# tanishqkumar/ssd

Measured on AMD Instinct MI355X. Metric: output tokens/sec + p50 TTFT, Llama-3-70B SSD k=7 f=3; mean accepted len, higher is better.
Workload: dtype bf16

## Files before the change

### ssd_amd/csrc/gemm_pf.hip

```cpp
#include "common.h"
#include <algorithm>
#include <cstdlib>

enum { PF_EPI_ROWS = 0, PF_EPI_SILU_FRAG = 1, PF_EPI_PARTIALS = 2 };

constexpr int PF_WAVES_DEFAULT = 4;
constexpr int PF_U = 4;

template <int MT, int NT, int UU, int DIRECT, int PF_WAVES, int BPS = 1, int BPRE = 0>
__global__ void __launch_bounds__(64 * PF_WAVES, PF_WAVES <= 4 ? 2 : 1)
gemm_pf_kernel(const u32x4_t* __restrict__ Wf, const u32x4_t* __restrict__ Xf, float* __restrict__ ws,
               int M, int N, int K, int kt_per_split, int mt_valid, const bf16_t* __restrict__ bias,
               void* __restrict__ Yv, int ldy) {
  __shared__ u32x4_t xs[2 * BPS][MT][64];
  constexpr int KTS = 16 + DIRECT;
  KTRACE(KTS, 0);
  constexpr int U = UU;
  static_assert(UU % (2 * BPS) == 0, "an even number of phases per unrolled pass");
  constexpr int FPW = (MT + PF_WAVES - 1) / PF_WAVES;
  const int lane = threadIdx.x & 63;
  const int wave = __builtin_amdgcn_readfirstlane(threadIdx.x >> 6);
  const int KT = K >> 5;
  const int g0 = (blockIdx.x * PF_WAVES + wave) * NT;
  const int kz0 = blockIdx.y * kt_per_split;
  const int nk = kt_per_split;

  f32x4_t acc[NT][MT];
#pragma unroll
  for (int nt = 0; nt < NT; ++nt)
#pragma unroll
    for (int mt = 0; mt < MT; ++mt) acc[nt][mt] = f32x4_t{0.f, 0.f, 0.f, 0.f};

  const u32x4_t* wp = Wf + (((size_t)g0 * KT + kz0) << 6) + lane;
  const size_t wstride = (size_t)KT << 6;
  const u32x4_t* xp[FPW];
  int xmt[FPW];
#pragma unroll
  for (int f = 0; f < FPW; ++f) {
    xmt[f] = wave + PF_WAVES * f;
    const int src = min(xmt[f], mt_valid - 1);
    xp[f] = Xf + (((size_t)src * KT + kz0) << 6) + lane;
  }

  u32x4_t a[U][NT], xr[2][BPS][FPW];
  auto load_w = [&](u32x4_t (&d)[NT], int kt) {
#pragma unroll
    for (int nt = 0; nt < NT; ++nt) d[nt] = __builtin_nontemporal_load(wp + nt * wstride + ((size_t)kt << 6));
  };
  auto load_x = [&](u32x4_t (&d)[FPW], int kt) {
#pragma unroll
    for (int f = 0; f < FPW; ++f) d[f] = xp[f][(size_t)kt << 6];
  };
  auto stage_x = [&](const u32x4_t (&d)[FPW], int slot) {
#pragma unroll
    for (int f = 0; f < FPW; ++f)
      if (xmt[f] < MT) xs[slot][xmt[f]][lane] = d[f];
  };
  auto compute = [&](const u32x4_t (&w)[NT], int slot) {
#pragma unroll
    for (int mt = 0; mt < MT; ++mt) {
      const u32x4_t b = xs[slot][mt][lane];
#pragma unroll
      for (int nt = 0; nt < NT; ++nt) acc[nt][mt] = mfma16(w[nt], b, acc[nt][mt]);
    }
  };

  const int klast = nk - 1;
#pragma unroll
  for (int b = 0; b < BPS; ++b) load_x(xr[0][b], b);
#pragma unroll
  for (int u = 0; u < U; ++u) load_w(a[u], u);
#pragma unroll
  for (int b = 0; b < BPS; ++b) load_x(xr[1][b], BPS + b);
#pragma unroll
  for (int b = 0; b < BPS; ++b) stage_x(xr[0][b], b);
#pragma unroll
  for (int b = 0; b < BPS; ++b) load_x(xr[0][b], min(2 * BPS + b, klast));
  KTRACE(KTS, 1);
  __syncthreads();
  KTRACE(KTS, 2);
  for (int kt = 0; kt < nk; kt += U) {
#pragma unroll
    for (int u = 0; u < U; u += BPS) {
      const int k = kt + u;
      const int par = (u / BPS) & 1;
#pragma unroll
      for (int b = 0; b < BPS; ++b) stage_x(xr[par ^ 1][b], (par ^ 1) * BPS + b);
#pragma unroll
      for (int b = 0; b < BPS; ++b) load_x(xr[par ^ 1][b], min(k + 3 * BPS + b, klast));
      if constexpr (BPRE == 2 && BPS == 2) {
        u32x4_t b0[MT], b1[MT];
#pragma unroll
        for (int mt = 0; mt < MT; ++mt) b0[mt] = xs[par * BPS][mt][lane];
#pragma unroll
        for (int mt = 0; mt < MT; ++mt) b1[mt] = xs[par * BPS + 1][mt][lane];
        __builtin_amdgcn_sched_barrier(0);
#pragma unroll
        for (int mt = 0; mt < MT; ++mt)
#pragma unroll
          for (int nt = 0; nt < NT; ++nt) acc[nt][mt] = mfma16(a[u][nt], b0[mt], acc[nt][mt]);
        load_w(a[u], min(k + U, klast));
#pragma unroll
        for (int mt = 0; mt < MT; ++mt)
#pragma unroll
          for (int nt = 0; nt < NT; ++nt) acc[nt][mt] = mfma16(a[u + 1][nt], b1[mt], acc[nt][mt]);
        load_w(a[u + 1], min(k + 1 + U, klast));
      } else {
#pragma unroll
        for (int b = 0; b < BPS; ++b) {
          compute(a[u + b], par * BPS + b);
          load_w(a[u + b], min(k + b + U, klast));
        }
      }
      __syncthreads();
    }
  }

  KTRACE(KTS, 3);
  const int mcol = lane & 15, nrow = (lane >> 4) * 4;
  if constexpr (DIRECT == 1) {
#pragma unroll
    for (int nt = 0; nt < NT; ++nt) {
      const int n = (g0 + nt) * 16 + nrow;
#pragma unroll
      for (int mt = 0; mt < MT; ++mt) {
        const int m = mt * 16 + mcol;
        f32x4_t s = acc[nt][mt];
        if (bias) {
#pragma unroll
          for (int r = 0; r < 4; ++r) s[r] += bf2f(bias[n + r]);
        }
        if (m < M) {
          const u32x2_t v = {pack_bf2(s[0], s[1]), pack_bf2(s[2], s[3])};
          *reinterpret_cast<u32x2_t*>(reinterpret_cast<bf16_t*>(Yv) + (size_t)m * ldy + n) = v;
        }
      }
    }
    KTRACE(KTS, 4);
    return;
  }
  if constexpr (DIRECT == 2) {
    const int KT2 = (N >> 1) >> 5;
    u32x2_t* out2 = reinterpret_cast<u32x2_t*>(Yv);
#pragma unroll
    for (int pr = 0; pr < NT / 2; ++pr) {
      const int f = ((g0 >> 1) + pr) * 16 + nrow;
      const int ng = (g0 + 2 * pr) * 16 + nrow, nu = ng + 16;
#pragma unroll
      for (int mt = 0; mt < MT; ++mt) {
        const int m = mt * 16 + mcol;
        float o[4];
#pragma unroll
        for (int r = 0; r < 4; ++r) {
          float gb = acc[2 * pr][mt][r], ub = acc[2 * pr + 1][mt][r];
          if (bias) { gb += bf2f(bias[ng + r]); ub += bf2f(bias[nu + r]); }
          gb = round_bf(gb); ub = round_bf(ub);
          o[r] = (gb / (1.0f + __expf(-gb))) * ub;
        }
        if (m < M) {
          const u32x2_t v = {pack_bf2(o[0], o[1]), pack_bf2(o[2], o[3])};
          out2[frag_chunk(m, f >> 3, KT2) * 2 + ((f >> 2) & 1)] = v;
        }
      }
    }
    KTRACE(KTS, 4);
    return;
  }
  float* out = ws + (size_t)blockIdx.y * M * N;
#pragma unroll
  for (int nt = 0; nt < NT; ++nt) {
    const int n = (g0 + nt) * 16 + nrow;
#pragma unroll
    for (int mt = 0; mt < MT; ++mt) {
      const int m = mt * 16 + mcol;
      if (m < M) *reinterpret_cast<f32x4_t*>(out + (size_t)m * N + n) = acc[nt][mt];
    }
  }
  KTRACE(KTS, 4);
}

template <int EPI>
__global__ void __launch_bounds__(256)
gemm_pf_epilogue_kernel(const float* __restrict__ ws, const bf16_t* __restrict__ bias, void* __restrict__ Yv,
                        int M, int N, int splits, int ldy) {
  const size_t MN = (size_t)M * N;
  if (EPI == PF_EPI_ROWS) {
    const size_t i4 = ((size_t)blockIdx.x * blockDim.x + threadIdx.x) * 4;
    if (i4 >= MN) return;
    const int m = (int)(i4 / N), n = (int)(i4 % N);
    f32x4_t s = *reinterpret_cast<const f32x4_t*>(ws + i4);
    for (int z = 1; z < splits; ++z) s += *reinterpret_cast<const f32x4_t*>(ws + z * MN + i4);
    if (bias) {
#pragma unroll
      for (int r = 0; r < 4; ++r) s[r] += bf2f(bias[n + r]);
    }
    const u32x2_t v = {pack_bf2(s[0], s[1]), pack_bf2(s[2], s[3])};
    *reinterpret_cast<u32x2_t*>(reinterpret_cast<bf16_t*>(Yv) + (size_t)m * ldy + n) = v;
  } else {
    const int half = N >> 1;
    const size_t i4 = ((size_t)blockIdx.x * blockDim.x + threadIdx.x) * 4;
    if (i4 >= (size_t)M * half) return;
    const int m = (int)(i4 / half), f = (int)(i4 % half);
    const int ng = ((f >> 4) * 2) * 16 + (f & 15), nu = ng + 16;
    f32x4_t g = *reinterpret_cast<const f32x4_t*>(ws + (size_t)m * N + ng);
    f32x4_t u = *reinterpret_cast<const f32x4_t*>(ws + (size_t)m * N + nu);
    for (int z = 1; z < splits; ++z) {
      g += *reinterpret_cast<const f32x4_t*>(ws + z * MN + (size_t)m * N + ng);
      u += *reinterpret_cast<const f32x4_t*>(ws + z * MN + (size_t)m * N + nu);
    }
    float o[4];
#pragma unroll
    for (int r = 0; r < 4; ++r) {
      float gb = g[r], ub = u[r];
      if (bias) { gb += bf2f(bias[ng + r]); ub += bf2f(bias[nu + r]); }
      gb = round_bf(gb); ub = round_bf(ub);
      o[r] = (gb / (1.0f + __expf(-gb))) * ub;
    }
    const u32x2_t v = {pack_bf2(o[0], o[1]), pack_bf2(o[2], o[3])};
    reinterpret_cast<u32x2_t*>(Yv)[frag_chunk(m, f >> 3, half >> 5) * 2 + ((f >> 2) & 1)] = v;
  }
}

template <int MT, int NT, int DIRECT>
static int pf_launch_d(const void* x, const void* w, float* ws, int M, int N, int K, int splits, const void* bias, void* y,
                       int ldy, int waves, int uu, int bps, int bpre, hipStream_t st) {
  const int KT = K >> 5;
  dim3 grid(N / (16 * NT * waves), splits);
  const int nk = KT / splits;
  if (uu <= 0) uu = (NT <= 2 && nk % 8 == 0) ? 8 : PF_U;
  if (nk % uu != 0 || bps < 1) return SSD_ERR_ARG;
  bool launched = false;
#define PF_GO_B(UU, WV, B, PRE)                                                                                          \
  if (!launched && uu == UU && waves == WV && bps == B && bpre == PRE) {                                                 \
    launched = true;                                                                                                     \
    hipLaunchKernelGGL((gemm_pf_kernel<MT, NT, UU, DIRECT, WV, B, PRE>), grid, dim3(64 * WV), 0, st, (const u32x4_t*)w, \
                       (const u32x4_t*)x, ws, M, N, K, nk, (M + 15) / 16, (const bf16_t*)bias, y, ldy);                  \
  }
#define PF_GO(UU, WV, B) PF_GO_B(UU, WV, B, 0)
  PF_GO(4, 4, 1)
  if constexpr (NT == 1 && MT == 8 && DIRECT != 2) {
    PF_GO(8, 4, 1) PF_GO(8, 4, 2) PF_GO(8, 8, 1) PF_GO(8, 8, 2)
  }
  if constexpr (NT == 2) {
    PF_GO(8, 4, 1) PF_GO(4, 8, 1) PF_GO(8, 8, 1)
    if constexpr (MT == 8) {
      PF_GO(8, 4, 2) PF_GO(8, 8, 2)
      PF_GO_B(8, 4, 2, 2) PF_GO_B(8, 8, 2, 2) PF_GO_B(8, 5, 2, 2)
      PF_GO(8, 3, 1) PF_GO(8, 3, 2) PF_GO(8, 5, 1) PF_GO(8, 5, 2) PF_GO(8, 6, 2) PF_GO(8, 7, 1) PF_GO(8, 7, 2)
    }
  }
#undef PF_GO
#undef PF_GO_B
  if (!launched) return SSD_ERR_ARG;
  return hipGetLastError() == hipSuccess ? SSD_OK : SSD_ERR_LAUNCH;
}

template <int MT, int NT>
static int pf_launch(const void* x, const void* w, float* ws, int M, int N, int K, int splits, int direct, const void* bias,
                     void* y, int ldy, int waves, int uu, int bps, int bpre, hipStream_t st) {
  if (direct == 1) return pf_launch_d<MT, NT, 1>(x, w, ws, M, N, K, splits, bias, y, ldy, waves, uu, bps, bpre, st);
  if (direct == 2) return pf_launch_d<MT, NT, 2>(x, w, ws, M, N, K, splits, bias, y, ldy, waves, uu, bps, bpre, st);
  return pf_launch_d<MT, NT, 0>(x, w, ws, M, N, K, splits, bias, y, ldy, waves, uu, bps, bpre, st);
}

static void pf_pick(int N, int K, int* nt_out, int* splits_out, int* waves_out = nullptr) {
  const int KT = K >> 5;
  int nt = 2, waves = 4, s = 1;
  if (N % (16 * 2 * 4) != 0) { *nt_out = 4; *splits_out = 1; if (waves_out) *waves_out = 4; return; }
  const int blocks4 = N / (16 * 2 * 4);
  if (blocks4 < 160) {
    while (s < 8 && (blocks4 * s < 160 || KT / s > 96)) s *= 2;
    while (s > 1 && KT % (s * PF_U) != 0) s /= 2;
  }
  if (N % (16 * 2 * 8) == 0 && (N / (16 * 2 * 8)) * s >= 160) waves = 8;
  *nt_out = nt; *splits_out = s;
  if (waves_out) *waves_out = waves;
}

static void pf_refine(int M, int N, int K, int splits, int* waves, int* bps) {
  *bps = 1;
  if (M <= 64) return;
  const int nk = (K >> 5) / splits;
  if (nk % 8 != 0) return;
  *bps = 2;
  if (N % (16 * 2 * 5) == 0 && ((N / (16 * 2 * 5)) * splits) % 256 == 0) *waves = 5;
}

typedef __attribute__((address_space(1))) void* lm_gptr_t;
typedef __attribute__((address_space(3))) void* lm_lptr_t;
constexpr int LM_MAX_M = 16384;
constexpr int LM_CUS = 256;

template <int BM, int BN, int WM, int WN, int DIRECT>
__global__ void __launch_bounds__(64 * WM * WN, 1)
gemm_lm_kernel(const u32x4_t* __restrict__ Wf, const u32x4_t* __restrict__ Xf, float* __restrict__ ws, int M, int N, int K,
               int nkb, int tiles_m, int tiles_n, const bf16_t* __restrict__ bias, void* __restrict__ Yv, int ldy) {
  constexpr int NW = WM * WN;
  constexpr int TW = BN / 16, TX = BM / 16, TT = TW + TX;
  constexpr int G = 2 * TT / NW;
  constexpr int MTW = TX / WM, NTW = TW / WN;
  static_assert((2 * TT) % NW == 0 && TX % WM == 0 && TW % WN == 0 && NTW % 2 == 0, "tile geometry");
  __shared__ u32x4_t lds[2][2][TT][64];
  const int lane = threadIdx.x & 63;
  const int wave = __builtin_amdgcn_readfirstlane(threadIdx.x >> 6);
  const int wm = wave / WN, wn = wave % WN;
  const int KT = K >> 5;

  const int nwg = gridDim.x, orig = blockIdx.x;
  const int q = nwg >> 3, r = nwg & 7, xcd = orig & 7;
  const int wgid = (xcd < r ? xcd * (q + 1) : r * (q + 1) + (xcd - r) * q) + (orig >> 3);
  const int tiles = tiles_m * tiles_n;
  const int z = wgid / tiles, t = wgid - z * tiles;
  const int mg0 = (t % tiles_m) * TX, ng0 = (t / tiles_m) * TW;
  const int mg_valid = (M + 15) >> 4, ng_valid = N >> 4;
  const int kt0 = z * nkb * 2;

  const u32x4_t* src[G];
#pragma unroll
  for (int i = 0; i < G; ++i) {
    const int j = wave * G + i, tt = j % TT, ks = j / TT;
    const int grp = tt < TW ? min(ng0 + tt, ng_valid - 1) : min(mg0 + tt - TW, mg_valid - 1);
    src[i] = (tt < TW ? Wf : Xf) + (((size_t)grp * KT + kt0 + ks) << 6) + lane;
  }
  auto issue = [&](int kb, int buf) {
#pragma unroll
    for (int i = 0; i < G; ++i) {
      const int j = wave * G + i;
      __builtin_amdgcn_global_load_lds((lm_gptr_t)(src[i] + ((size_t)kb << 7)), (lm_lptr_t)&lds[buf][j / TT][j % TT][0], 16, 0, 0);
    }
  };

  f32x4_t acc[NTW][MTW];
#pragma unroll
  for (int nt = 0; nt < NTW; ++nt)
#pragma unroll
    for (int mt = 0; mt < MTW; ++mt) acc[nt][mt] = f32x4_t{0.f, 0.f, 0.f, 0.f};

  issue(0, 0);
  for (int kb = 0; kb < nkb; ++kb) {
    const int cur = kb & 1;
    asm volatile("s_waitcnt vmcnt(0) lgkmcnt(0)" ::: "memory");
    __builtin_amdgcn_s_barrier();
    asm volatile("" ::: "memory");
    if (kb + 1 < nkb) issue(kb + 1, cur ^ 1);
#pragma unroll
    for (int ks = 0; ks < 2; ++ks) {
      u32x4_t a[NTW], b[MTW];
#pragma unroll
      for (int nt = 0; nt < NTW; ++nt) a[nt] = lds[cur][ks][wn * NTW + nt][lane];
#pragma unroll
      for (int mt = 0; mt < MTW; ++mt) b[mt] = lds[cur][ks][TW + wm * MTW + mt][lane];
#pragma unroll
      for (int mt = 0; mt < MTW; ++mt)
#pragma unroll
        for (int nt = 0; nt < NTW; ++nt) acc[nt][mt] = mfma16(a[nt], b[mt], acc[nt][mt]);
    }
  }

  const int mcol = lane & 15, nrow = (lane >> 4) * 4;
  const int gm0 = mg0 + wm * MTW, gn0 = ng0 + wn * NTW;
  if constexpr (DIRECT == 1) {
#pragma unroll
    for (int nt = 0; nt < NTW; ++nt) {
      if (gn0 + nt >= ng_valid) continue;
      const int n = (gn0 + nt) * 16 + nrow;
      float bv[4] = {0.f, 0.f, 0.f, 0.f};
      if (bias) {
#pragma unroll
        for (int r4 = 0; r4 < 4; ++r4) bv[r4] = bf2f(bias[n + r4]);
      }
#pragma unroll
      for (int mt = 0; mt < MTW; ++mt) {
        const int m = (gm0 + mt) * 16 + mcol;
        f32x4_t s = acc[nt][mt];
        if (bias) {
#pragma unroll
          for (int r4 = 0; r4 < 4; ++r4) s[r4] += bv[r4];
        }
        if (m < M) {
          const u32x2_t v = {pack_bf2(s[0], s[1]), pack_bf2(s[2], s[3])};
          *reinterpret_cast<u32x2_t*>(reinterpret_cast<bf16_t*>(Yv) + (size_t)m * ldy + n) = v;
        }
      }
    }
  } else if constexpr (DIRECT == 2) {
    const int KT2 = (N >> 1) >> 5;
    u32x2_t* out2 = reinterpret_cast<u32x2_t*>(Yv);
#pragma unroll
    for (int pr = 0; pr < NTW / 2; ++pr) {
      const int gg = gn0 + 2 * pr;
      if (gg >= ng_valid) continue;
      const int f = (gg >> 1) * 16 + nrow;
      const int ng = gg * 16 + nrow, nu = ng + 16;
#pragma unroll
      for (int mt = 0; mt < MTW; ++mt) {
        const int m = (gm0 + mt) * 16 + mcol;
        float o[4];
#pragma unroll
        for (int r4 = 0; r4 < 4; ++r4) {
          float gb = acc[2 * pr][mt][r4], ub = acc[2 * pr + 1][mt][r4];
          if (bias) { gb += bf2f(bias[ng + r4]); ub += bf2f(bias[nu + r4]); }
          gb = round_bf(gb); ub = round_bf(ub);
          o[r4] = (gb / (1.0f + __expf(-gb))) * ub;
        }
        if (m < M) {
          const u32x2_t v = {pack_bf2(o[0], o[1]), pack_bf2(o[2], o[3])};
          out2[frag_chunk(m, f >> 3, KT2) * 2 + ((f >> 2) & 1)] = v;
        }
      }
    }
  } else {
    float* out = ws + (size_t)z * M * N;
#pragma unroll
    for (int nt = 0; nt < NTW; ++nt) {
      if (gn0 + nt >= ng_valid) continue;
      const int n = (gn0 + nt) * 16 + nrow;
#pragma unroll
      for (int mt = 0; mt < MTW; ++mt) {
        const int m = (gm0 + mt) * 16 + mcol;
        if (m < M) *reinterpret_cast<f32x4_t*>(out + (size_t)m * N + n) = acc[nt][mt];
      }
    }
  }
}

constexpr int LM_FORMS = 4;
static const int lm_bm[LM_FORMS] = {256, 128, 256, 128}, lm_bn[LM_FORMS] = {256, 256, 128, 128}, lm_occ[LM_FORMS] = {1, 1, 1, 2};

static int64_t lm_tiles(int form, int M, int N) {
  return (int64_t)((M + lm_bm[form] - 1) / lm_bm[form]) * ((N + lm_bn[form] - 1) / lm_bn[form]);
}

static void lm_pick(int M, int N, int K, int* form_out, int* splits_out) {
  static const double rel[LM_FORMS] = {1.0, 0.8, 0.8, 0.8};
  int best = 0;
  double best_t = 0;
  for (int f = 0; f < LM_FORMS; ++f) {
    const int64_t per_round = (int64_t)LM_CUS * lm_occ[f];
    const double t = (double)((lm_tiles(f, M, N) + per_round - 1) / per_round) * lm_bm[f] * lm_bn[f] * lm_occ[f] / (65536.0 * rel[f]);
    if (f == 0 || t < best_t - 1e-9) { best = f; best_t = t; }
  }
  const int64_t cnt = lm_tiles(best, M, N), slots = (int64_t)LM_CUS * lm_occ[best];
  const int nkb = K / 64;
  int s = 1;
  if (cnt * 2 <= slots)
    while (s < 8 && cnt * s * 2 <= slots && nkb % (s * 2) == 0 && nkb / (s * 2) >= 8) s *= 2;
  *form_out = best + 1;
  *splits_out = s;
}

static int64_t lm_workspace(int M, int N, int K) {
  int form, s;
  lm_pick(M, N, K, &form, &s);
  return s > 1 ? (int64_t)s * M * N * 4 : 0;
}

template <int BM, int BN, int WM, int WN>
static int lm_go(const void* x, const void* w, float* ws, int M, int N, int K, int splits, int direct, const void* bias, void* y,
                 int ldy, hipStream_t st) {
  const int tiles_m = (M + BM - 1) / BM, tiles_n = (N + BN - 1) / BN;
  const int nkb = (K / 64) / splits;
  const dim3 grid((unsigned)(tiles_m * tiles_n * splits)), block(64 * WM * WN);
#define LM_ARGS (const u32x4_t*)w, (const u32x4_t*)x, ws, M, N, K, nkb, tiles_m, tiles_n, (const bf16_t*)bias, y, ldy
  if (direct == 1) hipLaunchKernelGGL((gemm_lm_kernel<BM, BN, WM, WN, 1>), grid, block, 0, st, LM_ARGS);
  else if (direct == 2) hipLaunchKernelGGL((gemm_lm_kernel<BM, BN, WM, WN, 2>), grid, block, 0, st, LM_ARGS);
  else hipLaunchKernelGGL((gemm_lm_kernel<BM, BN, WM, WN, 0>), grid, block, 0, st, LM_ARGS);
#undef LM_ARGS
  return hipGetLastError() == hipSuccess ? SSD_OK : SSD_ERR_LAUNCH;
}

static int lm_gemm(const void* x_frag, const void* w_frag, const void* bias, void* y, int M, int N, int K, int ldy, int epilogue,
                   void* workspace, int64_t workspace_bytes, int form, int splits, hipStream_t st) {
  if (M > LM_MAX_M || N <= 0 || K <= 0 || N % 128 != 0 || K % 128 != 0) return SSD_ERR_SHAPE;
  if (epilogue != PF_EPI_ROWS && epilogue != PF_EPI_SILU_FRAG) return SSD_ERR_ARG;
  if (form < 0 || form > LM_FORMS) return SSD_ERR_ARG;
  int dform, dsplits;
  lm_pick(M, N, K, &dform, &dsplits);
  if (form == 0) form = dform;
  if (splits <= 0) splits = dform == form ? dsplits : 1;
  if (splits > 16 || (K / 64) % splits != 0) return SSD_ERR_ARG;
  if (!x_frag || !w_frag || !y) return SSD_ERR_ARG;
  const int direct = splits == 1 ? (epilogue == PF_EPI_ROWS ? 1 : 2) : 0;
  if (!direct && (!workspace || workspace_bytes < (int64_t)splits * M * N * 4)) return SSD_ERR_ARG;
  float* ws = (float*)workspace;
  int rc;
#define LM_A x_frag, w_frag, ws, M, N, K, splits, direct, bias, y, ldy, st
  switch (form) {
    case 1: rc = lm_go<256, 256, 2, 4>(LM_A); break;
    case 2: rc = lm_go<128, 256, 2, 4>(LM_A); break;
    case 3: rc = lm_go<256, 128, 4, 2>(LM_A); break;
    default: rc = lm_go<128, 128, 2, 2>(LM_A); break;
  }
#undef LM_A
  if (rc != SSD_OK || direct) return rc;
  if (epilogue == PF_EPI_ROWS) {
    const size_t items = (size_t)M * N / 4;
    hipLaunchKernelGGL((gemm_pf_epilogue_kernel<PF_EPI_ROWS>), dim3((unsigned)((items + 255) / 256)), dim3(256), 0, st, ws,
                       (const bf16_t*)bias, y, M, N, splits, ldy);
  } else {
    const size_t items = (size_t)M * (N / 2) / 4;
    hipLaunchKernelGGL((gemm_pf_epilogue_kernel<PF_EPI_SILU_FRAG>), dim3((unsigned)((items + 255) / 256)), dim3(256), 0, st, ws,
                       (const bf16_t*)bias, y, M, N, splits, ldy);
  }
  return hipGetLastError() == hipSuccess ? SSD_OK : SSD_ERR_LAUNCH;
}

extern "C" int ssd_gemm_pf_workspace_bytes(int M, int N, int K, int64_t* bytes) {
  if (!bytes || M <= 0 || N <= 0 || K <= 0 || N % (16 * 2 * PF_WAVES_DEFAULT) != 0) return SSD_ERR_ARG;
  if (M > 128) {
    if (M > LM_MAX_M || K % 128 != 0) return SSD_ERR_ARG;
    int64_t need = 0;
    for (int m = 256;; m += 128) {
      const int mm = m < M ? m : M;
      need = std::max(need, lm_workspace(mm, N, K));
      if (mm == M) break;
    }
    *bytes = need;
    return SSD_OK;
  }
  int nt, splits;
  pf_pick(N, K, &nt, &splits);
  *bytes = (int64_t)splits * M * N * 4;
  return SSD_OK;
}

extern "C" int ssd_gemm_pf_cfg(const void* x_frag, const void* w_frag, const void* bias, void* y, int M, int N, int K,
                               int ldy, int epilogue, void* workspace, int64_t workspace_bytes, int nt, int splits,
                               void* stream) {
  if (M > 128) return lm_gemm(x_frag, w_frag, bias, y, M, N, K, ldy, epilogue, workspace, workspace_bytes, nt & 0xff, splits,
                              (hipStream_t)stream);
  if (M <= 16 || M > 128 || N <= 0 || K <= 0 || (K % (32 * PF_U))) return SSD_ERR_SHAPE;
  if (epilogue != PF_EPI_ROWS && epilogue != PF_EPI_SILU_FRAG && epilogue != PF_EPI_PARTIALS) return SSD_ERR_ARG;
  if (epilogue == PF_EPI_PARTIALS && bias) return SSD_ERR_ARG;
  int waves = (nt >> 8) & 0xff;
  const int uu = (nt >> 16) & 0xff;
  int bps = (nt >> 24) & 0xf;
  const int bpre = (nt >> 28) & 3;
  nt &= 0xff;
  if (waves == 0) waves = PF_WAVES_DEFAULT;
  if (bps == 0) bps = 1;
  if (nt != 1 && nt != 2 && nt != 4) return SSD_ERR_ARG;
  if (nt == 1 && (epilogue == PF_EPI_SILU_FRAG || M <= 64)) return SSD_ERR_ARG;
  if (waves != 4 && !(waves >= 3 && waves <= 8 && nt <= 2)) return SSD_ERR_ARG;
  if (N % (16 * nt * waves) != 0) return SSD_ERR_SHAPE;
  const int KT = K >> 5;
  if (splits <= 0) { int nt_d; pf_pick(N, K, &nt_d, &splits); if (nt_d != nt) splits = 1; }
  if (splits > 16) return SSD_ERR_ARG;
  if (KT % (splits * PF_U) != 0) return SSD_ERR_ARG;
  const int direct = (splits == 1 && epilogue != PF_EPI_PARTIALS) ? (epilogue == PF_EPI_ROWS ? 1 : 2) : 0;
  if (!direct && (!workspace || workspace_bytes < (int64_t)splits * M * N * 4)) return SSD_ERR_ARG;
  hipStream_t st = (hipStream_t)stream;
  float* ws = (float*)workspace;
  const int mt = (M + 15) / 16;
  int rc;
#define PF_ARGS x_frag, w_frag, ws, M, N, K, splits, direct, bias, y, ldy, waves, uu, bps, bpre, st
  if (mt <= 4) rc = nt == 4 ? pf_launch<4, 4>(PF_ARGS) : pf_launch<4, 2>(PF_ARGS);
  else rc = nt == 4 ? pf_launch<8, 4>(PF_ARGS) : nt == 2 ? pf_launch<8, 2>(PF_ARGS) : pf_launch<8, 1>(PF_ARGS);
#undef PF_ARGS
  if (rc != SSD_OK || direct || epilogue == PF_EPI_PARTIALS) return rc;
  if (epilogue == PF_EPI_ROWS) {
    const size_t items = (size_t)M * N / 4;
    hipLaunchKernelGGL((gemm_pf_epilogue_kernel<PF_EPI_ROWS>), dim3((unsigned)((items + 255) / 256)), dim3(256), 0, st, ws,
                       (const bf16_t*)bias, y, M, N, splits, ldy);
  } else {
    const size_t items = (size_t)M * (N / 2) / 4;
    hipLaunchKernelGGL((gemm_pf_epilogue_kernel<PF_EPI_SILU_FRAG>), dim3((unsigned)((items + 255) / 256)), dim3(256), 0, st,
                       ws, (const bf16_t*)bias, y, M, N, splits, ldy);
  }
  return hipGetLastError() == hipSuccess ? SSD_OK : SSD_ERR_LAUNCH;
}

extern "C" int ssd_gemm_pf(const void* x_frag, const void* w_frag, const void* bias, void* y, int M, int N, int K,
                           int ldy, int epilogue, void* workspace, int64_t workspace_bytes, int splits, void* stream) {
  if (N <= 0 || K <= 0 || N % (16 * 2 * PF_WAVES_DEFAULT) != 0) return SSD_ERR_SHAPE;
  if (M > 128) return lm_gemm(x_frag, w_frag, bias, y, M, N, K, ldy, epilogue, workspace, workspace_bytes, 0, splits, (hipStream_t)stream);
  int nt, s, waves, bps;
  pf_pick(N, K, &nt, &s, &waves);
  if (splits > 0) { s = splits; waves = 4; }
  if (s > 16 || (K >> 5) % s != 0) return SSD_ERR_ARG;
  pf_refine(M, N, K, s, &waves, &bps);
  const int bpre = (bps == 2 && nt == 2 && M > 64 && (waves == 4 || waves == 5 || waves == 8) && ((K >> 5) / s) % 8 == 0) ? 2 : 0;
  return ssd_gemm_pf_cfg(x_frag, w_frag, bias, y, M, N, K, ldy, epilogue, workspace, workspace_bytes,
                         nt | (waves << 8) | (bps << 24) | (bpre << 28), s, stream);
}

KT_DEFINE_SETTER(gemm_pf)
```

Measured before the change: 113.0.

## Add streaming multi-stage LDS ring GEMM kernel for under-occupied skinny GEMMs

Adds a new gemm_ps kernel that streams weight and activation tiles into a deep shared-memory ring buffer using direct global-to-LDS loads, with explicit vmcnt waits to keep several stages in flight. The default path now routes to it when the old config launches too few workgroups, choosing a tile width so the workgroup count is a multiple of the CU count. The intent is to raise memory-level parallelism and CU fill for bandwidth-bound small-M GEMMs. The epilogue store is also factored into a shared helper, and a probe script is added. The hand-tuned waitcnt accounting and the new shape selection could lower performance or break correctness on some shapes.

```diff
diff --git a/profiles/pf_stream_probe.py b/profiles/pf_stream_probe.py
--- /dev/null
+++ b/profiles/pf_stream_probe.py
@@ -0,0 +1,124 @@
+import argparse
+import ctypes as C
+import json
+import os
+import sys
+
+import torch
+
+ROOT = os.path.dirname(os.path.dirname(os.path.abspath(__file__)))
+sys.path.insert(0, ROOT)
+import ssd_amd.hip.lib as L
+
+if os.environ.get("SSD_PROBE_LIB"):
+    L.lib_path = lambda: os.environ["SSD_PROBE_LIB"]
+from ssd_amd.hip import ops as H
+
+BF = torch.bfloat16
+STREAM = 1 << 30
+SHAPES = [
+    ("70b.qkv", 10240, 8192, H.EPI_ROWS), ("70b.o", 8192, 8192, H.PF_EPI_PARTIALS),
+    ("70b.gate_up", 57344, 8192, H.EPI_SILU_FRAG), ("70b.down", 8192, 28672, H.PF_EPI_PARTIALS),
+    ("8b.gate_up", 28672, 4096, H.EPI_SILU_FRAG), ("8b.down", 4096, 14336, H.PF_EPI_PARTIALS),
+    ("qwen32b.qkv", 10240, 5120, H.EPI_ROWS), ("qwen32b.gate_up", 51200, 5120, H.EPI_SILU_FRAG),
+    ("qwen32b.down", 5120, 25600, H.PF_EPI_PARTIALS),
+]
+
+
+def old_default(M, N, K):
+    KT = K >> 5
+    waves, s = 4, 1
+    blocks4 = N // 128
+    if blocks4 < 160:
+        while s < 8 and (blocks4 * s < 160 or KT // s > 96):
+            s *= 2
+        while s > 1 and KT % (s * 4) != 0:
+            s //= 2
+    if N % 256 == 0 and (N // 256) * s >= 160:
+        waves = 8
+    bps = 1
+    if M > 64 and (KT // s) % 8 == 0:
+        bps = 2
+        if N % 160 == 0 and ((N // 160) * s) % 256 == 0:
+            waves = 5
+    bpre = 2 if (bps == 2 and M > 64 and waves in (4, 5, 8)) else 0
+    return 2 | (waves << 8) | (bps << 24) | (bpre << 28), s
+
+
+def call(lib, xf, w, y, ws, M, N, K, epi, nt, splits):
+    rc = lib.ssd_gemm_pf_cfg(xf.data_ptr(), w.data_ptr(), None, y.data_ptr(), M, N, K, N, epi, ws.data_ptr(),
+                             ws.numel() * 4, nt, splits, C.c_void_p(torch.cuda.current_stream().cuda_stream))
+    return rc
+
+
+def out_bytes(y, ws, M, N, epi, splits):
+    if epi == H.PF_EPI_PARTIALS:
+        return ws[: splits * M * N].view(torch.int32).clone()
+    return y.view(torch.int16).clone()
+
+
+@torch.inference_mode()
+def main():
+    ap = argparse.ArgumentParser()
+    ap.add_argument("--reps", type=int, default=20)
+    ap.add_argument("--m", type=int, nargs="+", default=[128])
+    ap.add_argument("--lm", action="store_true")
+    ap.add_argument("--shapes", nargs="+", default=None)
+    a = ap.parse_args()
+    lib = L.load_library()
+    lib.ssd_gemm_pf_cfg.restype = C.c_int
+    lib.ssd_gemm_pf_cfg.argtypes = [C.c_void_p, C.c_void_p, C.c_void_p, C.c_void_p, C.c_int, C.c_int, C.c_int, C.c_int, C.c_int,
+                                    C.c_void_p, C.c_int64, C.c_int, C.c_int, C.c_void_p]
+    for name, N, K, epi in SHAPES:
+        if a.shapes and name not in a.shapes:
+            continue
+        nbuf = max(3, -(-(2 << 30) // (2 * N * K)))
+        ws_ = [(torch.randn(N * K // 64, device="cuda") * 0.05).to(BF).repeat(64) for _ in range(nbuf)]
+        for M in a.m:
+            xf = (torch.randn(H.frag_numel(M, K), device="cuda") * 0.5).to(BF)
+            y = torch.zeros(M * N, device="cuda", dtype=BF)
+            wsb = torch.zeros(16 * M * N + 64, dtype=torch.float32, device="cuda")
+            nt0, s0 = old_default(M, N, K)
+            forms = [("old", nt0, s0)]
+            for tw in (16, 14, 12, 10, 8, 6):
+                if N % (16 * tw) == 0:
+                    forms.append((f"stream.tw{tw}", STREAM | (tw << 8), s0))
+                    if M > 64:
+                        forms.append((f"stream.tw{tw}.kpb1", STREAM | (tw << 8) | (1 << 24), s0))
+            forms.append(("default", None, 0))
+            if a.lm and M == 128:
+                forms += [("lm.128x256", (1 << 31) | 2, s0), ("lm.128x128", (1 << 31) | 4, s0)]
+            ref = None
+            for fname, nt, s in forms:
+                def go(i):
+                    if nt is None:
+                        H.gemm_pf(xf, ws_[i % nbuf], y, M, N, K, N, wsb, epilogue=epi)
+                        return 0
+                    return call(lib, xf, ws_[i % nbuf], y, wsb, M, N, K, epi, C.c_int32(nt & 0xffffffff).value, s)
+                y.zero_(); wsb.zero_()
+                rc = go(0)
+                if rc != 0:
+                    print(json.dumps({"matrix": name, "M": M, "form": fname, "rc": rc}), flush=True)
+                    continue
+                torch.cuda.synchronize()
+                got = out_bytes(y, wsb, M, N, epi, s0)
+                if ref is None:
+                    ref = got
+                same = bool(torch.equal(got, ref))
+                for i in range(3):
+                    go(i)
+                ev = [(torch.cuda.Event(enable_timing=True), torch.cuda.Event(enable_timing=True)) for _ in range(a.reps)]
+                for i, (e0, e1) in enumerate(ev):
+                    e0.record(); go(i + 1); e1.record()
+                torch.cuda.synchronize()
+                t = sorted(e0.elapsed_time(e1) * 1e3 for e0, e1 in ev)
+                us = t[len(t) // 2]
+                print(json.dumps({"matrix": name, "N": N, "K": K, "M": M, "form": fname, "nt": nt, "splits": s0, "us_p50": round(us, 1),
+                                  "us_min": round(t[0], 1), "tb_s": round(2 * N * K / us / 1e6, 2), "bit_identical_to_old": same}),
+                      flush=True)
+        del ws_
+        torch.cuda.empty_cache()
+
+
+if __name__ == "__main__":
+    main()
diff --git a/ssd_amd/csrc/gemm_pf.hip b/ssd_amd/csrc/gemm_pf.hip
--- a/ssd_amd/csrc/gemm_pf.hip
+++ b/ssd_amd/csrc/gemm_pf.hip
@@ -6,6 +6,66 @@
 
 constexpr int PF_WAVES_DEFAULT = 4;
 constexpr int PF_U = 4;
+
+template <int MT, int NT, int DIRECT>
+__device__ __forceinline__ void pf_store(const f32x4_t (&acc)[NT][MT], int g0, int lane, int M, int N, float* __restrict__ ws,
+                                         int z, const bf16_t* __restrict__ bias, void* __restrict__ Yv, int ldy) {
+  const int mcol = lane & 15, nrow = (lane >> 4) * 4;
+  if constexpr (DIRECT == 1) {
+#pragma unroll
+    for (int nt = 0; nt < NT; ++nt) {
+      const int n = (g0 + nt) * 16 + nrow;
+#pragma unroll
+      for (int mt = 0; mt < MT; ++mt) {
+        const int m = mt * 16 + mcol;
+        f32x4_t s = acc[nt][mt];
+        if (bias) {
+#pragma unroll
+          for (int r = 0; r < 4; ++r) s[r] += bf2f(bias[n + r]);
+        }
+        if (m < M) {
+          const u32x2_t v = {pack_bf2(s[0], s[1]), pack_bf2(s[2], s[3])};
+          *reinterpret_cast<u32x2_t*>(reinterpret_cast<bf16_t*>(Yv) + (size_t)m * ldy + n) = v;
+        }
+      }
+    }
+  } else if constexpr (DIRECT == 2) {
+    const int KT2 = (N >> 1) >> 5;
+    u32x2_t* out2 = reinterpret_cast<u32x2_t*>(Yv);
+#pragma unroll
+    for (int pr = 0; pr < NT / 2; ++pr) {
+      const int f = ((g0 >> 1) + pr) * 16 + nrow;
+      const int ng = (g0 + 2 * pr) * 16 + nrow, nu = ng + 16;
+#pragma unroll
+      for (int mt = 0; mt < MT; ++mt) {
+        const int m = mt * 16 + mcol;
+        float o[4];
+#pragma unroll
+        for (int r = 0; r < 4; ++r) {
+          float gb = acc[2 * pr][mt][r], ub = acc[2 * pr + 1][mt][r];
+          if (bias) { gb += bf2f(bias[ng + r]); ub += bf2f(bias[nu + r]); }
+          gb = round_bf(gb); ub = round_bf(ub);
+          o[r] = (gb / (1.0f + __expf(-gb))) * ub;
+        }
+        if (m < M) {
+          const u32x2_t v = {pack_bf2(o[0], o[1]), pack_bf2(o[2], o[3])};
+          out2[frag_chunk(m, f >> 3, KT2) * 2 + ((f >> 2) & 1)] = v;
+        }
+      }
+    }
+  } else {
+    float* out = ws + (size_t)z * M * N;
+#pragma unroll
+    for (int nt = 0; nt < NT; ++nt) {
+      const int n = (g0 + nt) * 16 + nrow;
+#pragma unroll
+      for (int mt = 0; mt < MT; ++mt) {
+        const int m = mt * 16 + mcol;
+        if (m < M) *reinterpret_cast<f32x4_t*>(out + (size_t)m * N + n) = acc[nt][mt];
+      }
+    }
+  }
+}
 
 template <int MT, int NT, int UU, int DIRECT, int PF_WAVES, int BPS = 1, int BPRE = 0>
 __global__ void __launch_bounds__(64 * PF_WAVES, PF_WAVES <= 4 ? 2 : 1)
@@ -117,65 +177,107 @@
   }
 
   KTRACE(KTS, 3);
-  const int mcol = lane & 15, nrow = (lane >> 4) * 4;
-  if constexpr (DIRECT == 1) {
-#pragma unroll
-    for (int nt = 0; nt < NT; ++nt) {
-      const int n = (g0 + nt) * 16 + nrow;
+  pf_store<MT, NT, DIRECT>(acc, g0, lane, M, N, ws, blockIdx.y, bias, Yv, ldy);
+  KTRACE(KTS, 4);
+}
+
+typedef __attribute__((address_space(1))) void* lm_gptr_t;
+typedef __attribute__((address_space(3))) void* lm_lptr_t;
+
+template <int MT, int TW, int KPB>
+struct PsGeom {
+  static constexpr int NW = TW / 2;
+  static constexpr int TT = TW + MT;
+  static constexpr int ST = 160 / TT < 8 ? 160 / TT : 8;
+  static constexpr int XPW = (MT + NW - 1) / NW;
+  static constexpr int L = 2 + XPW;
+  static constexpr int VM_STEADY = (ST - 2 * KPB) * L;
+  static_assert(TW % 2 == 0 && ST >= 2 * KPB + 1 && VM_STEADY <= 63, "stream geometry");
+};
+
+template <int MT, int TW, int DIRECT, int KPB>
+__global__ void __launch_bounds__(32 * TW, 1)
+gemm_ps_kernel(const u32x4_t* __restrict__ Wf, const u32x4_t* __restrict__ Xf, float* __restrict__ ws,
+               int M, int N, int K, int nk, int mt_valid, const bf16_t* __restrict__ bias, void* __restrict__ Yv, int ldy) {
+  using G = PsGeom<MT, TW, KPB>;
+  constexpr int NW = G::NW, TT = G::TT, ST = G::ST, XPW = G::XPW;
+  __shared__ u32x4_t ring[ST][TT][64];
+  constexpr int KTS = 19 + DIRECT;
+  KTRACE(KTS, 0);
+  const int lane = threadIdx.x & 63;
+  const int wave = __builtin_amdgcn_readfirstlane(threadIdx.x >> 6);
+  const int KT = K >> 5;
+  const int g0 = (blockIdx.x * NW + wave) * 2;
+  const int kz0 = blockIdx.y * nk;
+
+  const u32x4_t* wsrc = Wf + (((size_t)g0 * KT + kz0) << 6) + lane;
+  const size_t wstride = (size_t)KT << 6;
+  const u32x4_t* xsrc[XPW];
+  int xslot[XPW];
+#pragma unroll
+  for (int f = 0; f < XPW; ++f) {
+    const int mt = min(wave + NW * f, MT - 1);
+    xslot[f] = TW + mt;
+    xsrc[f] = Xf + (((size_t)min(mt, mt_valid - 1) * KT + kz0) << 6) + lane;
+  }
+  auto issue = [&](int kt, int slot) {
+    const size_t o = (size_t)kt << 6;
+    __builtin_amdgcn_global_load_lds((lm_gptr_t)(wsrc + o), (lm_lptr_t)&ring[slot][wave * 2][0], 16, 0, 2);
+    __builtin_amdgcn_global_load_lds((lm_gptr_t)(wsrc + wstride + o), (lm_lptr_t)&ring[slot][wave * 2 + 1][0], 16, 0, 2);
+#pragma unroll
+    for (int f = 0; f < XPW; ++f) __builtin_amdgcn_global_load_lds((lm_gptr_t)(xsrc[f] + o), (lm_lptr_t)&ring[slot][xslot[f]][0], 16, 0, 0);
+  };
+  auto wrap = [](int s) { return s >= ST ? s - ST : s; };
+
+  f32x4_t acc[2][MT];
+#pragma unroll
+  for (int nt = 0; nt < 2; ++nt)
+#pragma unroll
+    for (int mt = 0; mt < MT; ++mt) acc[nt][mt] = f32x4_t{0.f, 0.f, 0.f, 0.f};
+
+  const int pre = min(ST - KPB, nk);
+  for (int s = 0; s < pre; ++s) issue(s, s);
+  KTRACE(KTS, 1);
+  int slot = 0, nslot = ST - KPB;
+  for (int kt = 0; kt < nk; kt += KPB) {
+    if (kt + ST - 1 < nk) {
+      asm volatile("s_waitcnt vmcnt(%0) lgkmcnt(0)" ::"n"(G::VM_STEADY) : "memory");
+      __builtin_amdgcn_s_barrier();
+      asm volatile("" ::: "memory");
+#pragma unroll
+      for (int j = 0; j < KPB; ++j) issue(kt + ST - KPB + j, wrap(nslot + j));
+    } else {
+      asm volatile("s_waitcnt vmcnt(0) lgkmcnt(0)" ::: "memory");
+      __builtin_amdgcn_s_barrier();
+      asm volatile("" ::: "memory");
+#pragma unroll
+      for (int j = 0; j < KPB; ++j)
+        if (kt + ST - KPB + j < nk) issue(kt + ST - KPB + j, wrap(nslot + j));
+    }
+    if (kt == 0) KTRACE(KTS, 2);
+    u32x4_t a[KPB][2], b[KPB][MT];
+#pragma unroll
+    for (int j = 0; j < KPB; ++j) {
+      const int sl = wrap(slot + j);
+      a[j][0] = ring[sl][wave * 2][lane];
+      a[j][1] = ring[sl][wave * 2 + 1][lane];
+#pragma unroll
+      for (int mt = 0; mt < MT; ++mt) b[j][mt] = ring[sl][TW + mt][lane];
+    }
+    if constexpr (KPB > 1) __builtin_amdgcn_sched_barrier(0);
+#pragma unroll
+    for (int j = 0; j < KPB; ++j)
 #pragma unroll
       for (int mt = 0; mt < MT; ++mt) {
-        const int m = mt * 16 + mcol;
-        f32x4_t s = acc[nt][mt];
-        if (bias) {
-#pragma unroll
-          for (int r = 0; r < 4; ++r) s[r] += bf2f(bias[n + r]);
-        }
-        if (m < M) {
-          const u32x2_t v = {pack_bf2(s[0], s[1]), pack_bf2(s[2], s[3])};
-          *reinterpret_cast<u32x2_t*>(reinterpret_cast<bf16_t*>(Yv) + (size_t)m * ldy + n) = v;
-        }
-      }
-    }
-    KTRACE(KTS, 4);
-    return;
-  }
-  if constexpr (DIRECT == 2) {
-    const int KT2 = (N >> 1) >> 5;
-    u32x2_t* out2 = reinterpret_cast<u32x2_t*>(Yv);
-#pragma unroll
-    for (int pr = 0; pr < NT / 2; ++pr) {
-      const int f = ((g0 >> 1) + pr) * 16 + nrow;
-      const int ng = (g0 + 2 * pr) * 16 + nrow, nu = ng + 16;
-#pragma unroll
-      for (int mt = 0; mt < MT; ++mt) {
-        const int m = mt * 16 + mcol;
-        float o[4];
-#pragma unroll
-        for (int r = 0; r < 4; ++r) {
-          float gb = acc[2 * pr][mt][r], ub = acc[2 * pr + 1][mt][r];
-          if (bias) { gb += bf2f(bias[ng + r]); ub += bf2f(bias[nu + r]); }
-          gb = round_bf(gb); ub = round_bf(ub);
-          o[r] = (gb / (1.0f + __expf(-gb))) * ub;
-        }
-        if (m < M) {
-          const u32x2_t v = {pack_bf2(o[0], o[1]), pack_bf2(o[2], o[3])};
-          out2[frag_chunk(m, f >> 3, KT2) * 2 + ((f >> 2) & 1)] = v;
-        }
-      }
-    }
-    KTRACE(KTS, 4);
-    return;
-  }
-  float* out = ws + (size_t)blockIdx.y * M * N;
-#pragma unroll
-  for (int nt = 0; nt < NT; ++nt) {
-    const int n = (g0 + nt) * 16 + nrow;
-#pragma unroll
-    for (int mt = 0; mt < MT; ++mt) {
-      const int m = mt * 16 + mcol;
-      if (m < M) *reinterpret_cast<f32x4_t*>(out + (size_t)m * N + n) = acc[nt][mt];
-    }
-  }
+        acc[0][mt] = mfma16(a[j][0], b[j][mt], acc[0][mt]);
+        acc[1][mt] = mfma16(a[j][1], b[j][mt], acc[1][mt]);
+      }
+    slot = wrap(slot + KPB);
+    nslot = wrap(nslot + KPB);
+  }
+
+  KTRACE(KTS, 3);
+  pf_store<MT, 2, DIRECT>(acc, g0, lane, M, N, ws, blockIdx.y, bias, Yv, ldy);
   KTRACE(KTS, 4);
 }
 
@@ -286,8 +388,52 @@
   if (N % (16 * 2 * 5) == 0 && ((N / (16 * 2 * 5)) * splits) % 256 == 0) *waves = 5;
 }
 
-typedef __attribute__((address_space(1))) void* lm_gptr_t;
-typedef __attribute__((address_space(3))) void* lm_lptr_t;
+constexpr int PF_NT_STREAM = 1 << 30;
+static const int ps_tws[] = {16, 14, 12, 10, 8, 6};
+
+static bool ps_tw_ok(int tw) {
+  for (int t : ps_tws)
+    if (t == tw) return true;
+  return false;
+}
+
+static int pf_stream_pick(int N, int splits) {
+  for (int tw : ps_tws) {
+    if (N % (16 * tw) != 0) continue;
+    const int64_t wgs = (int64_t)(N / (16 * tw)) * splits;
+    if (wgs % 256 == 0) return tw;
+  }
+  return 0;
+}
+
+template <int MT, int TW, int KPB>
+static int ps_go(const void* x, const void* w, float* ws, int M, int N, int K, int splits, int direct, const void* bias, void* y,
+                 int ldy, hipStream_t st) {
+  const dim3 grid(N / (16 * TW), splits), block(32 * TW);
+#define PS_ARGS (const u32x4_t*)w, (const u32x4_t*)x, ws, M, N, K, (K >> 5) / splits, (M + 15) / 16, (const bf16_t*)bias, y, ldy
+  if (direct == 1) hipLaunchKernelGGL((gemm_ps_kernel<MT, TW, 1, KPB>), grid, block, 0, st, PS_ARGS);
+  else if (direct == 2) hipLaunchKernelGGL((gemm_ps_kernel<MT, TW, 2, KPB>), grid, block, 0, st, PS_ARGS);
+  else hipLaunchKernelGGL((gemm_ps_kernel<MT, TW, 0, KPB>), grid, block, 0, st, PS_ARGS);
+#undef PS_ARGS
+  return hipGetLastError() == hipSuccess ? SSD_OK : SSD_ERR_LAUNCH;
+}
+
+template <int MT, int KPB>
+static int ps_launch(int tw, const void* x, const void* w, float* ws, int M, int N, int K, int splits, int direct, const void* bias,
+                     void* y, int ldy, hipStream_t st) {
+#define PS_A x, w, ws, M, N, K, splits, direct, bias, y, ldy, st
+  switch (tw) {
+    case 16: return ps_go<MT, 16, KPB>(PS_A);
+    case 14: return ps_go<MT, 14, KPB>(PS_A);
+    case 12: return ps_go<MT, 12, KPB>(PS_A);
+    case 10: return ps_go<MT, 10, KPB>(PS_A);
+    case 8: return ps_go<MT, 8, KPB>(PS_A);
+    case 6: return ps_go<MT, 6, KPB>(PS_A);
+  }
+#undef PS_A
+  return SSD_ERR_ARG;
+}
+
 constexpr int LM_MAX_M = 16384;
 constexpr int LM_CUS = 256;
 
@@ -532,6 +678,30 @@
   if (M <= 16 || M > 128 || N <= 0 || K <= 0 || (K % (32 * PF_U))) return SSD_ERR_SHAPE;
   if (epilogue != PF_EPI_ROWS && epilogue != PF_EPI_SILU_FRAG && epilogue != PF_EPI_PARTIALS) return SSD_ERR_ARG;
   if (epilogue == PF_EPI_PARTIALS && bias) return SSD_ERR_ARG;
+  hipStream_t st = (hipStream_t)stream;
+  float* ws = (float*)workspace;
+  const int mt = (M + 15) / 16;
+  const int KT = K >> 5;
+  int rc, direct;
+  if (nt & PF_NT_STREAM) {
+    if (splits <= 0) { int nt_d; pf_pick(N, K, &nt_d, &splits); }
+    if (splits > 16 || KT % (splits * PF_U) != 0) return SSD_ERR_ARG;
+    int tw = (nt >> 8) & 0xff;
+    if (tw == 0) tw = pf_stream_pick(N, splits);
+    if (!ps_tw_ok(tw)) return SSD_ERR_ARG;
+    if (N % (16 * tw) != 0) return SSD_ERR_SHAPE;
+    direct = (splits == 1 && epilogue != PF_EPI_PARTIALS) ? (epilogue == PF_EPI_ROWS ? 1 : 2) : 0;
+    if (!direct && (!workspace || workspace_bytes < (int64_t)splits * M * N * 4)) return SSD_ERR_ARG;
+    if (!x_frag || !w_frag || (direct && !y)) return SSD_ERR_ARG;
+    int kpb = (nt >> 24) & 0xf;
+    if (kpb == 0) kpb = mt > 4 ? 2 : 1;
+    if (kpb != 1 && kpb != 2) return SSD_ERR_ARG;
+    if ((KT / splits) % kpb != 0) return SSD_ERR_ARG;
+#define PS_L x_frag, w_frag, ws, M, N, K, splits, direct, bias, y, ldy, st
+    if (mt <= 4) rc = kpb == 2 ? ps_launch<4, 2>(tw, PS_L) : ps_launch<4, 1>(tw, PS_L);
+    else rc = kpb == 2 ? ps_launch<8, 2>(tw, PS_L) : ps_launch<8, 1>(tw, PS_L);
+#undef PS_L
+  } else {
   int waves = (nt >> 8) & 0xff;
   const int uu = (nt >> 16) & 0xff;
   int bps = (nt >> 24) & 0xf;
@@ -543,20 +713,16 @@
   if (nt == 1 && (epilogue == PF_EPI_SILU_FRAG || M <= 64)) return SSD_ERR_ARG;
   if (waves != 4 && !(waves >= 3 && waves <= 8 && nt <= 2)) return SSD_ERR_ARG;
   if (N % (16 * nt * waves) != 0) return SSD_ERR_SHAPE;
-  const int KT = K >> 5;
   if (splits <= 0) { int nt_d; pf_pick(N, K, &nt_d, &splits); if (nt_d != nt) splits = 1; }
   if (splits > 16) return SSD_ERR_ARG;
   if (KT % (splits * PF_U) != 0) return SSD_ERR_ARG;
-  const int direct = (splits == 1 && epilogue != PF_EPI_PARTIALS) ? (epilogue == PF_EPI_ROWS ? 1 : 2) : 0;
+  direct = (splits == 1 && epilogue != PF_EPI_PARTIALS) ? (epilogue == PF_EPI_ROWS ? 1 : 2) : 0;
   if (!direct && (!workspace || workspace_bytes < (int64_t)splits * M * N * 4)) return SSD_ERR_ARG;
-  hipStream_t st = (hipStream_t)stream;
-  float* ws = (float*)workspace;
-  const int mt = (M + 15) / 16;
-  int rc;
 #define PF_ARGS x_frag, w_frag, ws, M, N, K, splits, direct, bias, y, ldy, waves, uu, bps, bpre, st
   if (mt <= 4) rc = nt == 4 ? pf_launch<4, 4>(PF_ARGS) : pf_launch<4, 2>(PF_ARGS);
   else rc = nt == 4 ? pf_launch<8, 4>(PF_ARGS) : nt == 2 ? pf_launch<8, 2>(PF_ARGS) : pf_launch<8, 1>(PF_ARGS);
 #undef PF_ARGS
+  }
   if (rc != SSD_OK || direct || epilogue == PF_EPI_PARTIALS) return rc;
   if (epilogue == PF_EPI_ROWS) {
     const size_t items = (size_t)M * N / 4;
@@ -579,6 +745,9 @@
   if (splits > 0) { s = splits; waves = 4; }
   if (s > 16 || (K >> 5) % s != 0) return SSD_ERR_ARG;
   pf_refine(M, N, K, s, &waves, &bps);
+  const int tw = (int64_t)(N / (16 * nt * waves)) * s < 192 ? pf_stream_pick(N, s) : 0;
+  if (tw) return ssd_gemm_pf_cfg(x_frag, w_frag, bias, y, M, N, K, ldy, epilogue, workspace, workspace_bytes, PF_NT_STREAM | (tw << 8),
+                                 s, stream);
   const int bpre = (bps == 2 && nt == 2 && M > 64 && (waves == 4 || waves == 5 || waves == 8) && ((K >> 5) / s) % 8 == 0) ? 2 : 0;
   return ssd_gemm_pf_cfg(x_frag, w_frag, bias, y, M, N, K, ldy, epilogue, workspace, workspace_bytes,
                          nt | (waves << 8) | (bps << 24) | (bpre << 28), s, stream);
```

New measurement: 112.8 (median of 3 runs). About the same (-0.2%).
